# LazyLatte/vortex-raytracing

Hardware: AMD Instinct MI355X
Metric: Mrays/s (primary+shadow) at 1920x1080, 1M-tri BVH (higher is better)
Workload: dtype f32; 1 GPU; configs[2]: Sponza-class 1048576 tris, 1920x1080, primary + 1 shadow ray per hit; frames_in_flight=2, frames_per_launch_group=5, parallelism=1 GPU: whole frames, 5 per set of launches (vxrt_render_batch), 2 sets in flight, world_size=1, bvh_nodes=726809, bvh_depth=13

## Files before the change

vortex-raytracing_amd/csrc/rt_accel.hip:

```cpp
#include <algorithm>
#include <cmath>
#include <cstdio>
#include <cstdlib>
#include <cstring>
#include <utility>
#include "rt_internal.h"
#include "bvh_quant.h"

__global__ void accel_nodes_kernel(const uint32_t* __restrict__ ref, uint32_t n_nodes, uint4* __restrict__ out, int is_tlas,
                                   const uint32_t* __restrict__ bases, const uint32_t* __restrict__ ends, uint32_t nb,
                                   uint32_t n_tris, uint32_t n_blas, uint32_t bias, uint32_t* status) {
  const uint32_t i = blockIdx.x * blockDim.x + threadIdx.x;
  if (i >= n_nodes) return;
  const uint32_t* w = ref + (size_t)i * RT_NODE_DWORDS;
  const uint32_t imask = w[3] >> 24, leftFirst = w[4], leafData = w[5];
  uint32_t base = 0, end = n_nodes;
  if (!is_tlas) {
    bool in = false;
    for (uint32_t j = 0; j < nb; ++j) if (i >= bases[j] && i < ends[j]) { base = bases[j]; end = ends[j]; in = true; }
    if (!in) return;
  }
  if (imask != (is_tlas ? 1u : 0u)) return;
  const bool leaf = is_tlas ? (leafData != 0xffffffffu) : (leafData != 0u);
  if (leaf) return;
// ... 491 lines not shown
      ok = hipGetLastError() == hipSuccess && hipStreamSynchronize(st) == hipSuccess &&
           hipMemcpy(&levels, d_depth + nc, 4, hipMemcpyDeviceToHost) == hipSuccess;
    }
    (void)hipFree(d_depth);
  }
  (void)hipFree(d_ranges); (void)hipFree(d_status); (void)hipFree(d_troot);
  if (!ok || (hstatus & STATUS_BAD_SCENE) != 0) { accel_free(a); return -1; }
  static const int shallow_env = [] { const char* e = getenv("VXRT_SHALLOW"); return e ? atoi(e) : -1; }();
  a->levels = levels;
  a->shallow = levels <= RT_SHALLOW_LEVELS && shallow_env != 0;
  a->dev.nodes_c = (const uint4*)a->nodes_c; a->dev.ref_tlas = (const uint32_t*)s->tlas; a->dev.n_tlas = s->n_tlas_nodes; a->dev.tri_w = (const float4*)a->tri_w;
  a->dev.blas_root = (const uint32_t*)a->blas_root; a->dev.tlas_root = troot;
  a->dev.ident_root = 0u;
  if (troot >= 0xC0000000u && troot < DESC_IDLE) {
    float m[12];
    static const bool ident_off = [] { const char* e = getenv("VXRT_IDENT_ROOT"); return e && e[0] == '0'; }();
    if (!ident_off && hipMemcpy(m, (const uint32_t*)s->blas + (size_t)(troot & PAYLOAD_MASK) * (RT_BLAS_STRIDE / 4) + 1, sizeof m, hipMemcpyDeviceToHost) == hipSuccess) {
      bool id = true;
      for (int i = 0; i < 12; ++i) id = id && m[i] == ((i % 5 == 0) ? 1.0f : 0.0f);
      a->dev.ident_root = id ? 1u : 0u;
    }
  }
  a->dev.exact_decode = (hstatus & STATUS_FMA_DECODE_DIFFERS) ? 1u : 0u;
  a->dev.ref_bvh = (const uint32_t*)s->bvh;
  a->dev.blas = (const uint32_t*)s->blas; a->dev.triEx = (const rt_triex_t*)s->triEx;
  a->dev.mat = (const rt_material_t*)s->mat; a->dev.tex = (const uint8_t*)s->tex;
  a->dev.top_img = (const uint4*)a->top_img; a->dev.n_top = n_top; a->dev.tlas_root_top = troot_top;
  a->dev.blas_root_top = n_top ? a->top_roots + 2 : (const uint32_t*)a->blas_root;
  if (getenv("VXRT_DEBUG")) fprintf(stderr, "[vxrt] accel: %u top-of-tree nodes staged for LDS (cap %u)\n", n_top, TOP_CAP);
  *out = a;
  return 0;
}

int vxrt_accel_destroy(vxrt_accel_t* a) {
  if (!a) return 0;
  accel_free(a);
  return 0;
}

uint64_t vxrt_accel_bytes(const vxrt_accel_t* a) {
  if (!a) return 0;
  return (uint64_t)a->ref.n_tlas_nodes * CNODE_VEC4 * 16 + (uint64_t)a->ref.n_bvh_nodes * CNODE_VEC4 * 16 +
         (uint64_t)a->ref.n_tris * WTRI_FLOATS * 4 + (uint64_t)a->ref.n_blas * 4;
}

int vxrt_accel_info(const vxrt_accel_t* a, uint32_t which, uint64_t* value) {
  if (!a || !value) return -1;
  switch (which) {
  case 0: *value = a->levels; return 0;
  case 1: *value = a->shallow ? 1u : 0u; return 0;
  case 2: *value = a->dev.ident_root; return 0;
  case 3: *value = a->dev.exact_decode; return 0;
  case 4: *value = a->alpha_on ? 1u : 0u; return 0;
  }
  return -1;
}

__global__ __launch_bounds__(256) void accel_alpha_tri_kernel(const rt_triex_t* __restrict__ triEx, uint32_t n_tris, const uint8_t* __restrict__ thr, uint32_t n_mats,
                                                             uint8_t* __restrict__ out) {
  const uint32_t t = blockIdx.x * blockDim.x + threadIdx.x;
  if (t >= n_tris) return;
  const uint32_t m = triEx[t].texId;
  out[t] = m < n_mats ? thr[m] : (uint8_t)0;
}

int vxrt_accel_set_alpha_test(vxrt_accel_t* a, const uint8_t* thresholds, uint32_t n_mats, void* stream) {
  hipStream_t st = (hipStream_t)stream;
  if (!a || a->stale) return -1;
  const vxrt_scene_t& s = a->ref;
  bool any = false;
  if (thresholds) {
    if (n_mats != s.n_mats) return -1;
    for (uint32_t m = 0; m < n_mats; ++m) any = any || thresholds[m] != 0;
  }
  if (any) {
    if (!s.triEx || !s.mat || !s.tex) return -1;
    std::vector<rt_material_t> mats(n_mats);
    if (hipStreamSynchronize(st) != hipSuccess || hipMemcpy(mats.data(), s.mat, (size_t)n_mats * sizeof(rt_material_t), hipMemcpyDeviceToHost) != hipSuccess) return -1;
    for (uint32_t m = 0; m < n_mats; ++m)
      if (thresholds[m] != 0 && mats[m].diffuse_tex_id < 0) return -1;
    if (!a->alpha_mat && hipMalloc((void**)&a->alpha_mat, std::max<size_t>(s.n_mats, 16)) != hipSuccess) return -1;
    if (!a->alpha_tri && hipMalloc((void**)&a->alpha_tri, std::max<size_t>(s.n_tris, 16)) != hipSuccess) return -1;
  }
  for (uint32_t k = 0; k < MAX_FRAMES_IN_FLIGHT; ++k) {
    FrameCtx& c = a->ctx[k];
    if (!c.busy || c.last_stream == st) continue;
    if (c.done_recorded) { if (hipStreamWaitEvent(st, c.ev_done, 0) != hipSuccess) return -1; }
    else if (hipDeviceSynchronize() != hipSuccess) return -1;
  }
  if (any) {
    if (hipMemcpyAsync(a->alpha_mat, thresholds, n_mats, hipMemcpyHostToDevice, st) != hipSuccess) return -1;
    hipLaunchKernelGGL(accel_alpha_tri_kernel, dim3((s.n_tris + 255) / 256), dim3(256), 0, st, (const rt_triex_t*)s.triEx, s.n_tris,
                       (const uint8_t*)a->alpha_mat, n_mats, a->alpha_tri);
    if (hipGetLastError() != hipSuccess) { a->alpha_on = false; (void)hipStreamSynchronize(st); return -1; }
  }
  if (hipStreamSynchronize(st) != hipSuccess) { a->alpha_on = false; return -1; }
  a->alpha_on = any;
  return 0;
}

int vxrt_accel_frames_in_flight(vxrt_accel_t* a, uint32_t n) {
  if (!a || n < 1 || n > MAX_FRAMES_IN_FLIGHT) return -1;
  if (hipDeviceSynchronize() != hipSuccess) return -1;
  a->n_ctx = n; a->next_ctx = 0;
  return 0;
}
// ... 180 lines not shown
```

vortex-raytracing_amd/csrc/rt_internal.h:

```cpp
#pragma once
#include <hip/hip_runtime.h>
#include <stdint.h>
#include <vector>
#include "rt_types.h"
#include "../../include/vortex_hip.h"

#define STATUS_STACK_OVERFLOW 1u
#define STATUS_ITER_LIMIT 2u
#define STATUS_BAD_SCENE 4u
#define STATUS_FMA_DECODE_DIFFERS 8u

struct SceneDev {
  const uint4* nodes_c;
  const uint32_t* ref_tlas;
  uint32_t n_tlas;
  const float4* tri_w;
  const uint32_t* blas_root;
  uint32_t tlas_root;
  uint32_t exact_decode;
  const uint32_t* ref_bvh;
  const uint32_t* blas;
  const rt_triex_t* triEx;
  const rt_material_t* mat;
  const uint8_t* tex;
// ... 14 lines not shown
  uint64_t hitbuf_pixels = 0;
  uint32_t* defer = nullptr;
  uint64_t defer_cap = 0;
  uint32_t* ctl = nullptr;
  ShadeParams* pbatch = nullptr;
  float* cam = nullptr; uint64_t cam_floats = 0;
  bool ctl_dirty = false;
  struct Level {
    float* rays = nullptr; HitRec* hits = nullptr; uint32_t* parent = nullptr; float4* term = nullptr; float* col = nullptr;
    float* srays = nullptr; float* stmax = nullptr; HitRec* shits = nullptr;
    uint64_t cap = 0; uint32_t n = 0;
  };
  std::vector<Level> lv;
  uint32_t* bcount = nullptr;
  struct Lpt { uint32_t* cost = nullptr; uint32_t* order = nullptr; uint32_t cap = 0; uint32_t key[6] = {0, 0, 0, 0, 0, 0}; bool valid = false; };
  Lpt lpt[VXRT_MAX_BATCH + 1];
  float4* ao_geo = nullptr; float4* ao_nrm = nullptr; float4* ao_col = nullptr; uint32_t* ao_cnt = nullptr;
  uint32_t* ao_list = nullptr; uint32_t* ao_hdr = nullptr;
  float* ao_rays = nullptr; float* ao_tmax = nullptr; HitRec* ao_hits = nullptr; uint64_t ao_cap = 0, ao_ray_cap = 0;
  uint32_t* bin_hist = nullptr; uint32_t* bin_keys = nullptr; uint32_t* bin_order = nullptr; uint64_t bin_cap = 0, bin_ray_cap = 0;
  void* pool_spill = nullptr; uint64_t pool_spill_bytes = 0;
  hipStream_t side = nullptr;
  hipEvent_t ev_in = nullptr, ev_side = nullptr, ev_done = nullptr;
  bool busy = false, inited = false, done_recorded = false;
  hipStream_t last_stream = nullptr;
};

struct vxrt_accel {
  SceneDev dev{};
  vxrt_scene_t ref{};
  void* nodes_c = nullptr; void* tri_w = nullptr; void* blas_root = nullptr;
  void* top_img = nullptr; uint32_t* top_roots = nullptr;
  FrameCtx ctx[MAX_FRAMES_IN_FLIGHT];
  uint32_t n_ctx = 1, next_ctx = 0;
  bool stream_seen = false, multi_stream = false; hipStream_t first_stream = nullptr;
  float* uvtab = nullptr;
  uint32_t uv_w = 0, uv_h = 0;
  uint32_t* apriori = nullptr;
  uint32_t* batch_order[VXRT_MAX_BATCH + 1] = {}; uint32_t bo_tiles = 0;
  uint32_t ap_count = 0, ap_key[6] = {0, 0, 0, 0, 0, 0};
  uint64_t ap_cap = 0;
  float max_reflectivity = 0.0f;
  unsigned long long* trace_wave_log = nullptr;
  unsigned long long* end_log = nullptr;
  uint32_t levels = 0;
  bool shallow = false;
  int device = 0;
  struct RefitPlan* refit = nullptr;
  uint32_t blas_status = 0;
  bool stale = false;
  uint8_t* alpha_mat = nullptr; uint8_t* alpha_tri = nullptr;
  bool alpha_on = false;
};
```

vortex-raytracing_amd/csrc/rt_kernels.hip:

```cpp
#include <hip/hip_runtime.h>
#include <stdint.h>
#include "rt_internal.h"
#include "pinhole.h"

__device__ __forceinline__ float std_min(float a, float b) { return (b < a) ? b : a; }
__device__ __forceinline__ float std_max(float a, float b) { return (a < b) ? b : a; }

template <bool EXACT>
__device__ __forceinline__ float slab_interval(float tx1, float tx2, float ty1, float ty2, float tz1, float tz2) {
  float tmin, tmax;
  if (EXACT) {
    tmin = std_min(tx1, tx2);
    tmax = std_max(tx1, tx2);
    tmin = std_max(tmin, std_min(ty1, ty2));
    tmax = std_min(tmax, std_max(ty1, ty2));
    tmin = std_max(tmin, std_min(tz1, tz2));
    tmax = std_min(tmax, std_max(tz1, tz2));
  } else {
    tmin = fmaxf(fmaxf(fminf(tx1, tx2), fminf(ty1, ty2)), fminf(tz1, tz2));
    tmax = fminf(fminf(fmaxf(tx1, tx2), fmaxf(ty1, ty2)), fmaxf(tz1, tz2));
  }
  return (tmax < tmin || tmax <= 0) ? RT_LARGE_FLOAT : tmin;
}

// ... 342 lines not shown
#ifndef RT_QUEUE_DRY_MASK
#define RT_QUEUE_DRY_MASK 1
#endif
#ifndef RT_STEAL_SPREAD
#define RT_STEAL_SPREAD 0
#endif
#ifndef QUEUE_SHARDS
#define QUEUE_SHARDS 8u
#endif
#define QUEUE_STRIDE 32u
#define CTL_QUEUE_DWORDS (QUEUE_SHARDS * QUEUE_STRIDE)
#define CTL_DWORDS (32u + 3u * CTL_QUEUE_DWORDS)
#ifndef RT_WAVES_TRACE
#define RT_WAVES_TRACE 7
#endif
#ifndef RT_LDS_STACK_TRACE
#define RT_LDS_STACK_TRACE 7
#endif
#ifndef RT_WAVES_RENDER
#define RT_WAVES_RENDER 7
#endif
#ifndef RT_LDS_STACK_RENDER
#define RT_LDS_STACK_RENDER 6
#endif
#ifndef RT_WAVES_RENDER_PACKED
#define RT_WAVES_RENDER_PACKED 8
#endif
#ifndef RT_LDS_STACK_RENDER_PACKED
#define RT_LDS_STACK_RENDER_PACKED 5
#endif
#ifndef LDS_STACK
#define LDS_STACK 8
#endif
#ifndef RT_WG_WAVES
#define RT_WG_WAVES 4
#endif
#define RT_WG_THREADS (64 * RT_WG_WAVES)

enum { JOB_RENDER = 0, JOB_RENDER_SHADOW = 1, JOB_TRACE = 2, JOB_RENDER_GI = 3, JOB_TRACE_UNORDERED = 4 };
__host__ __device__ constexpr bool is_trace_job(int job) { return job == JOB_TRACE || job == JOB_TRACE_UNORDERED; }
enum { JOB_CAM = 8 };
__host__ __device__ constexpr int job_base(int job) { return job & ~JOB_CAM; }
__host__ __device__ constexpr bool is_cam_job(int job) { return (job & JOB_CAM) != 0; }
#ifndef RT_WAVES_GI
#define RT_WAVES_GI 7
#endif
#ifndef RT_LDS_STACK_GI
#define RT_LDS_STACK_GI 6
#endif
#ifndef RT_GI_DEAD_MAX
#define RT_GI_DEAD_MAX 64
#endif

#ifdef RT_ISA_MARKS
#define RT_MARK(name) asm volatile("; RTMARK " name)
#else
#define RT_MARK(name)
#endif

__device__ __forceinline__ size_t hit_index(uint32_t x, uint32_t lr, uint32_t tiles_x) {
  return ((size_t)(lr >> 3) * tiles_x + (x >> 3)) * 64u + ((lr & 7u) << 3) + (x & 7u);
}
__device__ __forceinline__ uint32_t frame_row(uint32_t lr, uint32_t y0, uint32_t row_step) { return y0 + (lr >> 3) * row_step + (lr & 7u); }

struct FastDiv { uint32_t d, m, s; };
static FastDiv fast_div_make(uint32_t d) {
  FastDiv f{d ? d : 1u, 1u, 0u};
  while ((1ull << f.s) < f.d) ++f.s;
  f.m = (uint32_t)((((1ull << f.s) - f.d) << 32) / f.d) + 1u;
  return f;
}
__device__ __forceinline__ uint32_t fast_div(uint32_t x, const FastDiv& f) { return (__umulhi(x, f.m) + x) >> f.s; }

struct PersistArgs {
  uint32_t W, H, y0, y1, tiles_x;
  FastDiv div_tiles_x, div_frame_tiles;
  uint32_t row_step;
  uint32_t total;
  const uint32_t* total_dev;
  HitRec* hits;
  const float* rays; const float* tmax; int any_hit;
  const uint32_t* order;
  unsigned long long* counters;
  uint32_t* status;
  uint32_t* queue;
  uint32_t per_shard;
  const float* utab; const float* vtab;
  uint32_t* defer_count; uint32_t* defer_list; uint32_t defer_cap;
  const uint32_t* tile_order; uint32_t* tile_cost;
  uint32_t shard_rot;
  unsigned long long* wave_log;
  unsigned long long* end_log;
  const ShadeParams* pbatch; uint32_t frame_tiles;
  uint32_t* dst; float* colors; uint32_t gi_seed;
  const uint8_t* alpha_tri;
};

#define RT_FAST_INV_MAX 0x1p+64f
#define RT_FAST_POS_MAX 0x1p+60f
__device__ __forceinline__ bool ray_in_fast_domain(float ox, float oy, float oz, float ix, float iy, float iz) {
  return fabsf(ix) <= RT_FAST_INV_MAX && fabsf(iy) <= RT_FAST_INV_MAX && fabsf(iz) <= RT_FAST_INV_MAX && ix != 0.0f && iy != 0.0f && iz != 0.0f &&
         fabsf(ox) <= RT_FAST_POS_MAX && fabsf(oy) <= RT_FAST_POS_MAX && fabsf(oz) <= RT_FAST_POS_MAX;
}

__device__ __forceinline__ float vmax_nonan(float a, float b) { float r; asm("v_max_f32 %0, %1, %2" : "=v"(r) : "v"(a), "v"(b)); return r; }

#define F_FOUND 1u
#define F_ANYHIT 2u
#define F_SHADOW 8u
#define F_WORLD 16u
#define F_RESUMED 32u

template <int JOB, int STATS, bool LDEXP, bool EXACT, bool PACKED = false, bool SHALLOW = false, bool ALPHA = false>
__global__ __launch_bounds__(EXACT ? 256 : RT_WG_THREADS, EXACT ? 4 : (is_trace_job(JOB) ? RT_WAVES_TRACE : (job_base(JOB) == JOB_RENDER_GI ? RT_WAVES_GI : (PACKED ? RT_WAVES_RENDER_PACKED : RT_WAVES_RENDER)))) void rt_persistent_kernel(SceneDev sc, ShadeParams p, PersistArgs A) {
  static_assert(!ALPHA || (STATS == 0 && !PACKED && !SHALLOW && job_base(JOB) != JOB_RENDER_GI), "alpha instantiations: see ALPHA above");
  constexpr int LSTK = EXACT ? LDS_STACK : (is_trace_job(JOB) ? RT_LDS_STACK_TRACE : (job_base(JOB) == JOB_RENDER_GI ? RT_LDS_STACK_GI : (PACKED ? RT_LDS_STACK_RENDER_PACKED : RT_LDS_STACK_RENDER)));
  constexpr int WG_WAVES = EXACT ? 4 : RT_WG_WAVES;
  constexpr bool USE_TOP = RT_TOP_NODES > 0 && !EXACT && !LDEXP;
  constexpr uint32_t DEAD_MAX = is_trace_job(JOB) ? RT_TRACE_DEAD_MAX : (job_base(JOB) == JOB_RENDER_GI ? RT_GI_DEAD_MAX : RT_DEAD_MAX);
  constexpr uint32_t FINISH_MIN = job_base(JOB) == JOB_RENDER_SHADOW ? RT_SHADOW_FINISH_MIN : 65u;
  const uint32_t lane = threadIdx.x & 63u;
  const uint32_t n_jobs = EXACT ? min(*A.defer_count, A.defer_cap) : (A.total_dev ? min(*A.total_dev, A.total) : A.total);
  const uint32_t per_shard = (EXACT || A.total_dev) ? (((n_jobs + QUEUE_SHARDS - 1) / QUEUE_SHARDS + 63u) & ~63u) : A.per_shard;

  __shared__ uint2 s_stk[WG_WAVES][LSTK][64];
  constexpr int NCTX = (!EXACT && is_trace_job(JOB)) ? 8 : 9;
  __shared__ uint32_t s_ctx[WG_WAVES][NCTX][64];
  __shared__ uint32_t s_dry;
  if (threadIdx.x == 0) s_dry = 0u;
  float* s_cam = nullptr;
  if constexpr (is_cam_job(JOB)) {
    s_cam = cam_lds<CAM_TAB>();
    for (uint32_t i = threadIdx.x; i < (uint32_t)CAM_TAB; i += blockDim.x) s_cam[i] = A.utab[i];
  }
  __syncthreads();
  uint2* const lstk = &s_stk[threadIdx.x >> 6][0][lane];
  uint32_t* const ctx = &s_ctx[threadIdx.x >> 6][0][lane];
#define CTX(i) ctx[((NCTX == 8 && (i) > 5) ? (i) - 1 : (i)) * 64]
  __shared__ uint4 s_top[USE_TOP ? 4 : 1][USE_TOP ? RT_TOP_NODES : 1];
  constexpr bool TRI_LDS = RT_TRI_LDS > 0 && !EXACT && !is_trace_job(JOB);
  __shared__ float4 s_tri[TRI_LDS ? WG_WAVES : 1][TRI_LDS ? 3 * RT_TRI_LDS : 1];
  const uint32_t n_top = USE_TOP ? min(sc.n_top, (uint32_t)RT_TOP_NODES) : 0u;
  if (USE_TOP && n_top) {
    for (uint32_t i = threadIdx.x; i < 4u * n_top; i += (uint32_t)(64 * WG_WAVES)) s_top[i / n_top][i % n_top] = sc.top_img[(size_t)(i / n_top) * RT_TOP_NODES + (i % n_top)];
    __syncthreads();
  }
  const uint32_t root_desc = (USE_TOP && n_top) ? sc.tlas_root_top : sc.tlas_root;
  const uint32_t* const blas_roots = (USE_TOP && n_top) ? sc.blas_root_top : sc.blas_root;
  const uint32_t root_blas_desc = is_inst_desc(root_desc) ? blas_roots[root_desc & PAYLOAD_MASK] : DESC_DONE;

  float arx = 0, ary = 0, arz = 0, aix = 0, aiy = 0, aiz = 0;
  float hitd = 0, path_m = 0, tos_m = 0;
  uint32_t cur = DESC_IDLE, tos_d = DESC_DONE, job = 0, flags = 0;
  float g_col[3] = {0.f, 0.f, 0.f}, g_alb[3] = {0.f, 0.f, 0.f}, g_ray[6] = {0.f, 0.f, 0.f, 0.f, 0.f, 0.f};
  int sp = 0;
  constexpr int STACK_CAP = SHALLOW ? 3 * RT_SHALLOW_LEVELS : LSTK + RT_STACK_ENTRIES;
  static_assert(STACK_CAP > LSTK, "stack");
  uint32_t ovf_d[STACK_CAP - LSTK];
  float ovf_m[STACK_CAP - LSTK];
  bool queue_empty = false;
  const uint32_t xcc_id = RT_XCC_HOME ? (uint32_t)__builtin_amdgcn_s_getreg((3 << 11) | (0 << 6) | 20) : blockIdx.x;
  const uint32_t shard = (xcc_id + A.shard_rot) % QUEUE_SHARDS;
  uint32_t tries = 0, loc_next = 0, loc_end = 0;
  uint32_t loc_off = 0;
  uint32_t lpt_tile = 0xFFFFFFFFu, lpt_work = 0; unsigned long long lpt_t0 = 0;
  Fetches fx;
  unsigned nrays = 0, nhit = 0;
  unsigned long long t_first = 0;
// ... 70 lines not shown
    for (int i = 0; i < 13; ++i) bw[i] = bp[i];
    if (STATS) { fx.node++; fx.inst++; }
    const float m00 = __uint_as_float(bw[1]), m01 = __uint_as_float(bw[2]), m02 = __uint_as_float(bw[3]), m03 = __uint_as_float(bw[4]);
    const float m10 = __uint_as_float(bw[5]), m11 = __uint_as_float(bw[6]), m12 = __uint_as_float(bw[7]), m13 = __uint_as_float(bw[8]);
    const float m20 = __uint_as_float(bw[9]), m21 = __uint_as_float(bw[10]), m22 = __uint_as_float(bw[11]), m23 = __uint_as_float(bw[12]);
    arx = m00 * ox + m01 * oy + m02 * oz + m03;
    ary = m10 * ox + m11 * oy + m12 * oz + m13;
    arz = m20 * ox + m21 * oy + m22 * oz + m23;
    const float cdx = m00 * dx + m01 * dy + m02 * dz;
    const float cdy = m10 * dx + m11 * dy + m12 * dz;
    const float cdz = m20 * dx + m21 * dy + m22 * dz;
    aix = 1.0f / cdx; aiy = 1.0f / cdy; aiz = 1.0f / cdz;
    const bool s2 = ray_in_fast_domain(arx, ary, arz, aix, aiy, aiz);
    if (!EXACT && !s2) { defer(true); return; }
    flags &= ~F_WORLD;
    CTX(0) = __float_as_uint(cdx); CTX(1) = __float_as_uint(cdy); CTX(2) = __float_as_uint(cdz);
    CTX(8) = blasIdx;
    cur = blas_roots[blasIdx];
  };
  auto start_ray = [&](float ox, float oy, float oz, float dx, float dy, float dz, float tmax_, bool any_) {
    arx = ox; ary = oy; arz = oz;
    aix = 1.0f / dx; aiy = 1.0f / dy; aiz = 1.0f / dz;
    const bool safe = ray_in_fast_domain(ox, oy, oz, aix, aiy, aiz);
    flags = (flags & (F_SHADOW | F_RESUMED)) | F_WORLD | (any_ ? F_ANYHIT : 0u);
    if (!EXACT && !safe) {
      if (!is_trace_job(JOB) && !is_cam_job(JOB) && !(flags & F_SHADOW)) cur = DESC_IDLE; else defer(false);
      return;
    }
    hitd = tmax_ > RT_LARGE_FLOAT ? RT_LARGE_FLOAT : tmax_;
    path_m = -__builtin_inff(); sp = 0; tos_d = DESC_DONE;
    cur = root_desc;
    nrays++;
    if (is_inst_desc(root_desc)) {
      const bool no_neg_zero = __float_as_uint(ox) != 0x80000000u && __float_as_uint(oy) != 0x80000000u && __float_as_uint(oz) != 0x80000000u;
      if (sc.ident_root && safe && no_neg_zero) {
        if (STATS) { fx.node++; fx.inst++; }
        flags &= ~F_WORLD;
        CTX(0) = __float_as_uint(dx); CTX(1) = __float_as_uint(dy); CTX(2) = __float_as_uint(dz);
        CTX(8) = root_desc & PAYLOAD_MASK;
        cur = root_blas_desc;
      } else enter_instance(root_desc & PAYLOAD_MASK, ox, oy, oz, dx, dy, dz);
    }
  };
  volatile uint32_t* const vovf_d = ovf_d;
  volatile float* const vovf_m = ovf_m;
  auto push = [&](uint32_t d, float m) {
    if (tos_d != DESC_DONE) {
      if (sp < LSTK) lstk[sp * 64] = make_uint2(tos_d, __float_as_uint(tos_m));
      else { ovf_d[sp - LSTK] = tos_d; ovf_m[sp - LSTK] = tos_m; }
      ++sp;
    }
    tos_d = d; tos_m = m;
  };
  auto pop_next = [&]() {
    cur = DESC_DONE;
    while (tos_d != DESC_DONE) {
      const uint32_t d = tos_d;
      const float m = tos_m;
      if (sp > 0) {
        --sp;
        if (sp < LSTK) { const uint2 e = lstk[sp * 64]; tos_d = e.x; tos_m = __uint_as_float(e.y); }
        else { tos_d = ovf_d[sp - LSTK]; tos_m = ovf_m[sp - LSTK]; }
      } else {
        tos_d = DESC_DONE;
      }
      if (m < hitd) { cur = d; path_m = m; break; }
    }
  };

  for (;;) {
    RT_MARK("fetch");
    if (STATS && A.wave_log) wl_tmark = __builtin_readcyclecounter();
    {
      const unsigned long long idle = __ballot(cur == DESC_IDLE);
      if (!queue_empty && idle != 0ull && (is_trace_job(JOB) || FINISH_MIN > 64u || idle == ~0ull || RT_DEAD_MAX < 64)) {
        const uint32_t wl_tries0 = tries; const unsigned long long wl_tpoll0 = (STATS && A.wave_log) ? __builtin_readcyclecounter() : 0ull;
        if (loc_next == loc_end) {
          uint32_t dry = RT_QUEUE_DRY_MASK ? *(volatile uint32_t*)&s_dry : 0u;
          while (tries < QUEUE_SHARDS) {
            const uint32_t step = RT_STEAL_SPREAD ? (((tries & 1u) << 2) | (tries & 2u) | ((tries >> 2) & 1u)) : tries;
            const uint32_t sid = (shard + step) % QUEUE_SHARDS;
            if (RT_QUEUE_DRY_MASK && ((dry >> sid) & 1u)) { ++tries; continue; }
            const uint32_t s_lo = sid * per_shard;
            uint32_t in_range;
            asm volatile("s_cmp_lt_u32 %1, %2\n\ts_cselect_b32 %0, 1, 0 ; RTGUARD shard_range" : "=s"(in_range)
                         : "s"(__builtin_amdgcn_readfirstlane(s_lo)), "s"(__builtin_amdgcn_readfirstlane(n_jobs)) : "scc");
            if (!in_range) { ++tries; continue; }
            const uint32_t s_n = min(per_shard, n_jobs - s_lo);
            uint32_t base = 0;
            constexpr uint32_t CHUNK = (is_trace_job(JOB) && !EXACT) ? (uint32_t)RT_TRACE_CHUNK : (uint32_t)RT_CHUNK;
            if (lane == 0) base = atomicAdd(A.queue + sid * QUEUE_STRIDE, CHUNK);
            base = __shfl(base, 0);
            if (base < s_n) {
              loc_next = s_lo + base; loc_end = s_lo + min(base + CHUNK, s_n);
              break;
            }
            if (RT_QUEUE_DRY_MASK) {
              if (lane == 0) atomicOr(&s_dry, 1u << sid);
              dry |= 1u << sid;
            }
            ++tries;
          }
          if (tries >= QUEUE_SHARDS) { queue_empty = true; if (STATS && A.wave_log && !wl_tq) wl_tq = wall_clock64(); }
          if (STATS && A.wave_log && !USE_TOP && tries != wl_tries0 && lane == 0) wl_no23 += (unsigned)(__builtin_readcyclecounter() - wl_tpoll0);
        }
        uint32_t avail = loc_end - loc_next;
        if (!is_trace_job(JOB) && !EXACT) {
// ... 23 lines not shown
            job = loc_next + rank + loc_off;
            flags = 0;
            if (!EXACT && is_trace_job(JOB) && A.order) job = A.order[job];
            if (EXACT) {
              const uint32_t wd = A.defer_list[job];
              job = wd & 0x7fffffffu;
              if (wd >> 31) { flags = F_SHADOW | F_RESUMED; if (job_base(JOB) == JOB_RENDER_SHADOW) CTX(5) = __float_as_uint(hit_slot()->dist); }
            }
            float ox, oy, oz, dx, dy, dz, tm;
            if (is_trace_job(JOB)) {
              world_ray(ox, oy, oz, dx, dy, dz, tm);
              start_ray(ox, oy, oz, dx, dy, dz, tm, A.any_hit != 0);
            } else {
              uint32_t x, y;
              pixel_of(job, x, y);
              if (x < A.W && y < A.y1) {
                world_ray(ox, oy, oz, dx, dy, dz, tm);
                start_ray(ox, oy, oz, dx, dy, dz, tm, (flags & F_SHADOW) != 0u);
              }
            }
          }
        }
        loc_next += min(avail, (uint32_t)__popcll(idle));
      }
      if (__ballot(cur != DESC_IDLE) == 0ull) {
        if (queue_empty && loc_next == loc_end) {
          if (!is_trace_job(JOB) && !EXACT && A.tile_cost && lane == 0 && lpt_tile != 0xFFFFFFFFu) {
            A.tile_cost[lpt_tile] = lpt_work;
            if (STATS && A.wave_log) A.tile_cost[2u * (A.total >> 6) + lpt_tile] = (uint32_t)min(wall_clock64() - lpt_t0, 0xFFFFFFFFull);
          }
          break;
        }
        if (STATS && A.wave_log) wl_tf += __builtin_readcyclecounter() - wl_tmark;
        continue;
      }
    }
    if (STATS && A.wave_log) wl_tf += __builtin_readcyclecounter() - wl_tmark;

    for (;;) {
      RT_MARK("loop_top");
      if (!is_trace_job(JOB) && !EXACT) ++lpt_work;
      if (STATS && A.wave_log) {
        const unsigned long long nm = __ballot(is_node_desc(cur));
        ++wl_iter;
        if (nm) {
          ++wl_node_x; wl_node_l += (unsigned)__popcll(nm);
          const uint32_t c0 = __shfl(cur, __ffsll((long long)nm) - 1);
          if (__ballot(is_node_desc(cur) && cur == c0) == nm) ++wl_no3;
        }
      }
      if (STATS && A.wave_log) wl_t0 = __builtin_readcyclecounter();
      RT_MARK("node");
      if (is_node_desc(cur)) {
        const bool top = (cur >> 30) == DK_TLAS;
        if (top && !(flags & F_WORLD)) {
          float ox, oy, oz, dx, dy, dz, tm;
          world_ray(ox, oy, oz, dx, dy, dz, tm);
          arx = ox; ary = oy; arz = oz; aix = 1.0f / dx; aiy = 1.0f / dy; aiz = 1.0f / dz;
          flags |= F_WORLD;
        }
        const uint32_t ni = cur & PAYLOAD_MASK;
        uint4 q0, q1, q2, q3;
        if (USE_TOP && (cur & DESC_TOP_FLAG)) {
          typedef uint32_t u32x4_t __attribute__((ext_vector_type(4)));
          typedef __attribute__((address_space(3))) const volatile u32x4_t lds_u32x4_t;
          lds_u32x4_t* tp = (lds_u32x4_t*)&s_top[0][0] + (cur & DESC_TOP_SLOT);
          const u32x4_t t0 = tp[0], t1 = tp[RT_TOP_NODES], t2 = tp[2 * RT_TOP_NODES], t3 = tp[3 * RT_TOP_NODES];
          q0 = make_uint4(t0.x, t0.y, t0.z, t0.w); q1 = make_uint4(t1.x, t1.y, t1.z, t1.w);
          q2 = make_uint4(t2.x, t2.y, t2.z, t2.w); q3 = make_uint4(t3.x, t3.y, t3.z, t3.w);
          if (STATS && A.wave_log) ++wl_no23;
        } else {
          const uint4* np = sc.nodes_c + (size_t)ni * CNODE_VEC4;
          q0 = np[0]; q1 = np[1]; q2 = np[2]; q3 = np[3];
        }
        const uint32_t* ref_node = nullptr;
        if (LDEXP) ref_node = top ? sc.ref_tlas + (size_t)ni * RT_NODE_DWORDS : sc.ref_bvh + (size_t)(ni - sc.n_tlas) * RT_NODE_DWORDS;
        if (STATS) fx.node++;
        Cand c[4];
        eval_children<EXACT, LDEXP>(q0, q1, q2, q3, ref_node, arx, ary, arz, aix, aiy, aiz, hitd, c);
        if (((job_base(JOB) == JOB_RENDER_SHADOW && RT_UNORDERED_OCCLUSION) || JOB == JOB_TRACE_UNORDERED) && STATS != 1 && __all((flags & F_ANYHIT) != 0u)) {
          const bool v0 = c[0].d < __builtin_inff(), v1 = c[1].d < __builtin_inff(), v2 = c[2].d < __builtin_inff(), v3 = c[3].d < __builtin_inff();
          if (v0 || v1 || v2 || v3) {
            bool more = true;
            if (sp + 4 > STACK_CAP) { atomicOr(A.status, STATUS_STACK_OVERFLOW); more = false; }
            cur = v0 ? c[0].desc : (v1 ? c[1].desc : (v2 ? c[2].desc : c[3].desc));
            if (more) {
              if (v1 && v0) push(c[1].desc, c[1].d);
              if (v2 && (v0 || v1)) push(c[2].desc, c[2].d);
              if (v3 && (v0 || v1 || v2)) push(c[3].desc, c[3].d);
            }
          } else {
            pop_next();
          }
        } else {
          order_children(c);
          if (c[0].d < __builtin_inff()) {
            bool more = true;
            if (sp + 4 > STACK_CAP) { atomicOr(A.status, STATUS_STACK_OVERFLOW); more = false; }
            if (more && c[3].d < __builtin_inff()) push(c[3].desc, vmax_nonan(path_m, c[3].d));
            if (more && c[2].d < __builtin_inff()) push(c[2].desc, vmax_nonan(path_m, c[2].d));
            if (more && c[1].d < __builtin_inff()) push(c[1].desc, vmax_nonan(path_m, c[1].d));
            cur = c[0].desc;
            path_m = vmax_nonan(path_m, c[0].d);
          } else {
            pop_next();
          }
        }
      }
      if (STATS && A.wave_log) { const unsigned long long t1 = __builtin_readcyclecounter(); wl_tn += t1 - wl_t0; wl_t0 = t1; }
      RT_MARK("inst");
      if (__any(is_inst_desc(cur))) {
        if (is_inst_desc(cur)) {
          float ox, oy, oz, dx, dy, dz, tm;
          world_ray(ox, oy, oz, dx, dy, dz, tm);
          enter_instance(cur & PAYLOAD_MASK, ox, oy, oz, dx, dy, dz);
        }
      }
      RT_MARK("leaf");
      const unsigned long long leafm = __ballot(is_leaf_desc(cur));
      if (leafm != 0ull && ((uint32_t)__popcll(leafm) >= (is_trace_job(JOB) ? RT_TRACE_LEAF_MIN : RT_LEAF_MIN) || __ballot(is_node_desc(cur) || is_inst_desc(cur)) == 0ull)) {
        if (STATS && A.wave_log) { ++wl_leaf_x; wl_leaf_l += (unsigned)__popcll(leafm); }
        if (!is_trace_job(JOB) && !EXACT) lpt_work += 2u;
        {
          bool tri_from_lds = false;
          if (TRI_LDS) {
            const uint32_t L0 = __shfl(cur, __ffsll((long long)leafm) - 1);
            const uint32_t c0 = (L0 >> LEAF_FIRST_BITS) & LEAF_MAX_INLINE;
            const unsigned long long same = __ballot(cur == L0);
            if (c0 != 0u && c0 <= (uint32_t)RT_TRI_LDS && (uint32_t)__popcll(same) >= (uint32_t)RT_TRI_LDS_MIN) {
              if (lane < 3u * c0) s_tri[threadIdx.x >> 6][lane] = sc.tri_w[(size_t)(L0 & LEAF_FIRST_MASK) * 3 + lane];
              tri_from_lds = cur == L0;
              if (STATS && A.wave_log) wl_no23 += (unsigned)__popcll(same);
            }
          }
          if (is_leaf_desc(cur)) {
            if (STATS) fx.node++;
            uint32_t leftFirst = cur & LEAF_FIRST_MASK, triCount = (cur >> LEAF_FIRST_BITS) & LEAF_MAX_INLINE;
            if (triCount == 0u) {
              const uint32_t* rn = sc.ref_bvh + (size_t)leftFirst * RT_NODE_DWORDS;
              leftFirst = rn[4]; triCount = rn[5];
            }
            const float cdx = __uint_as_float(CTX(0)), cdy = __uint_as_float(CTX(1)), cdz = __uint_as_float(CTX(2));
            bool stop = false;
            constexpr bool PREFETCH = is_trace_job(JOB) && RT_TRI_PREFETCH;
            float4 n0 = make_float4(0.f, 0.f, 0.f, 0.f), n1 = n0, n2 = n0;
            if (PREFETCH) { const float4* tp0 = sc.tri_w + (size_t)leftFirst * 3; n0 = tp0[0]; n1 = tp0[1]; n2 = tp0[2]; }
            for (uint32_t i = 0; i < triCount; ++i) {
              const uint32_t triIdx = leftFirst + i;
              float4 t0, t1, t2;
              if (TRI_LDS && tri_from_lds) {
                typedef float f32x4_t __attribute__((ext_vector_type(4)));
                typedef __attribute__((address_space(3))) const volatile f32x4_t lds_f32x4_t;
                lds_f32x4_t* lp = (lds_f32x4_t*)&s_tri[threadIdx.x >> 6][0] + 3u * i;
                const f32x4_t a0 = lp[0], a1 = lp[1], a2 = lp[2];
                t0 = make_float4(a0.x, a0.y, a0.z, a0.w); t1 = make_float4(a1.x, a1.y, a1.z, a1.w); t2 = make_float4(a2.x, a2.y, a2.z, a2.w);
              } else
              if (PREFETCH) {
                t0 = n0; t1 = n1; t2 = n2;
                if (i + 1u < triCount) { const float4* tn = sc.tri_w + (size_t)(triIdx + 1u) * 3; n0 = tn[0]; n1 = tn[1]; n2 = tn[2]; }
              } else {
                const float4* tp = sc.tri_w + (size_t)triIdx * 3;
                t0 = tp[0]; t1 = tp[1]; t2 = tp[2];
              }
              if (STATS) fx.tri++;
              float bx, by, bz;
              const float d = ray_tri(arx, ary, arz, cdx, cdy, cdz, t0, t1, t2, bx, by, bz);
              if (d < hitd) {
                if constexpr (ALPHA) { if (alpha_rejects(sc, A.alpha_tri, triIdx, bx, by, bz)) continue; }
                hitd = d;
                flags |= F_FOUND;
                if (!(job_base(JOB) == JOB_RENDER_SHADOW && (flags & F_SHADOW))) { CTX(3) = __float_as_uint(bx); CTX(4) = __float_as_uint(by); CTX(6) = CTX(8); CTX(7) = triIdx; }
                if (flags & F_ANYHIT) { stop = true; break; }
                if (!(path_m < hitd)) break;
              }
            }
            if (stop) { sp = 0; tos_d = DESC_DONE; cur = DESC_DONE; }
            else pop_next();
          }
        }
      }
      if (STATS && A.wave_log) { const unsigned long long t1 = __builtin_readcyclecounter(); wl_tl += t1 - wl_t0; }
      RT_MARK("loop_exit");
      const unsigned long long work = __ballot(is_work_desc(cur));
      if (work == 0ull) break;
      const unsigned long long done = __ballot(cur == DESC_DONE);
      const uint32_t n_done = (uint32_t)__popcll(done);
      const uint32_t n_idle = queue_empty && loc_next == loc_end ? 0u : 64u - (uint32_t)__popcll(work | done);
      if (n_done + n_idle >= DEAD_MAX || n_done >= FINISH_MIN) break;
    }

    RT_MARK("finish");
    if (STATS && A.wave_log) wl_tmark = __builtin_readcyclecounter();
    if (cur == DESC_DONE) {
      const bool found = (flags & F_FOUND) != 0u;
      HitRec h; h.dist = RT_LARGE_FLOAT; h.bx = 0; h.by = 0; h.bz = 0; h.blasIdx = 0; h.triIdx = 0;
      if (is_trace_job(JOB)) {
        if (found) {
          h.dist = hitd; h.bx = __uint_as_float(CTX(3)); h.by = __uint_as_float(CTX(4)); h.bz = 1 - h.bx - h.by;
          h.blasIdx = CTX(6); h.triIdx = CTX(7);
        }
        if (RT_TRACE_NT) {
          uint32_t* hp = (uint32_t*)hit_slot();
          __builtin_nontemporal_store(__float_as_uint(h.dist), hp); __builtin_nontemporal_store(__float_as_uint(h.bx), hp + 1);
          __builtin_nontemporal_store(__float_as_uint(h.by), hp + 2); __builtin_nontemporal_store(__float_as_uint(h.bz), hp + 3);
          __builtin_nontemporal_store(h.blasIdx, hp + 4); __builtin_nontemporal_store(h.triIdx, hp + 5);
        } else *hit_slot() = h;
        cur = DESC_IDLE;
      } else if (job_base(JOB) == JOB_RENDER_GI) {
        uint32_t x, y;
        pixel_of(job, x, y);
        const size_t e = (size_t)x + (size_t)y * A.W;
        bool write = false;
        float cr = 0.f, cg = 0.f, cb = 0.f;
        if (found) {
          h.dist = hitd; h.bx = __uint_as_float(CTX(3)); h.by = __uint_as_float(CTX(4)); h.bz = 1 - h.bx - h.by;
          h.blasIdx = CTX(6); h.triIdx = CTX(7);
        }
        if (!(flags & F_SHADOW)) {
          float ox, oy, oz, dx, dy, dz;
          pixel_ray(x, y, ox, oy, oz, dx, dy, dz);
          if (!found) {
            cr = p.bg[0]; cg = p.bg[1]; cb = p.bg[2];
            write = true;
          } else {
            float r, g, b, refl, Ix, Iy, Iz, Nx, Ny, Nz, a3[3];
            shade_terms<false>(sc, p, ox, oy, oz, dx, dy, dz, h, false, r, g, b, refl, Ix, Iy, Iz, Nx, Ny, Nz, nullptr, a3);
            float thr = 1.0f;
            thr *= refl;
            g_col[0] = r + p.bg[0] * thr; g_col[1] = g + p.bg[1] * thr; g_col[2] = b + p.bg[2] * thr;
            g_alb[0] = a3[0]; g_alb[1] = a3[1]; g_alb[2] = a3[2];
            ao_sample_ray(x, y, A.W, 1u, 0u, A.gi_seed, Ix, Iy, Iz, Nx, Ny, Nz, dx, dy, dz, g_ray);
            flags = F_SHADOW;
            start_ray(g_ray[0], g_ray[1], g_ray[2], g_ray[3], g_ray[4], g_ray[5], RT_LARGE_FLOAT, false);
          }
        } else {
          float r, g, b;
          shade_eval<false>(sc, p, g_ray[0], g_ray[1], g_ray[2], g_ray[3], g_ray[4], g_ray[5], h, found, false, r, g, b);
// ... 1244 lines not shown
    if (!upload_batch(a, c, r, t, s)) return false;
    A.pbatch = c->pbatch; A.tile_order = a->batch_order[r.batch];
  }
  if (!grow_device({{(void**)&c->defer, sizeof(uint32_t)}}, &c->defer_cap, A.total, GrowSync::STREAM, s)) return false;
  A.defer_count = c->ctl; A.defer_list = c->defer; A.defer_cap = A.total;
  A.queue = c->ctl + 32;
  A.per_shard = ((A.total + QUEUE_SHARDS - 1) / QUEUE_SHARDS + 63u) & ~63u;
  A.shard_rot = host_knobs().shard_rot;
  A.alpha_tri = a->alpha_on ? a->alpha_tri : nullptr;
  if (lpt && !ensure_lpt_tables(c, r, n_tiles, A, s)) return false;
  return r.cams || ensure_apriori(a, r, t, s);
}

struct LaunchPlan {
  bool lpt;
  bool packed;
  bool side_launch;
  uint32_t side_wgs;
  bool side_reserve;
  uint32_t grid_div;
  bool grid_div_small;
};
static LaunchPlan launch_plan(const vxrt_accel* a, const RenderRequest& r, uint32_t n_tiles, bool lpt, uint32_t ap_count) {
  const HostKnobs& k = host_knobs();
  LaunchPlan plan;
  plan.lpt = lpt;
  plan.packed = k.packed >= 0 ? k.packed != 0 : ((a->n_ctx > 1 || (k.packed_batch && r.batch > 1)) && n_tiles >= LPT_MIN_TILES);
  plan.side_launch = ap_count != 0;
  plan.side_wgs = plan.side_launch ? std::min<uint32_t>(EXACT_GRID, (ap_count + 255u) / 256u) : 0u;
  plan.side_reserve = k.side_reserve >= 0 ? k.side_reserve != 0 : a->n_ctx == 1;
  plan.grid_div = k.grid_div > 0 ? (uint32_t)k.grid_div : ((k.grid_div == 0 && a->n_ctx > 1) ? a->n_ctx : 1u);
  plan.grid_div_small = k.grid_div == 0;
  return plan;
}

template <class K>
static uint32_t main_grid(K kernel, const LaunchPlan& plan, uint32_t total) {
  const uint32_t side_wgs_r = plan.side_reserve ? plan.side_wgs : 0u;
  uint32_t g = persistent_grid(kernel, total + (uint64_t)side_wgs_r * RT_WG_THREADS);
  const uint32_t cap = persistent_grid(kernel, ~0ull >> 8);
  const uint32_t div = (plan.grid_div_small && (uint64_t)total >= 2ull * 64ull * RT_WG_WAVES * cap) ? 1u : plan.grid_div;
  if (div > 1u) g = std::min<uint32_t>(g, std::max<uint32_t>(cap / div, 1u));
  return std::max<uint32_t>(1u, g > side_wgs_r ? g - side_wgs_r : 1u);
}

struct FrameLaunch {
  const vxrt_accel* a; FrameCtx* c; const LaunchPlan& plan; const ShadeParams& p; hipStream_t s;
  PersistArgs A, X, X0;
};

template <int JOB, int STATS, bool PACKED, bool ALPHA = false>
static void launch_traversal(const FrameLaunch& l) {
  static_assert(!(PACKED && (job_base(JOB) == JOB_RENDER_GI || STATS != 0)), "only the timed render jobs have a packed form");
  with_decode_and_depth<STATS == 0 && !ALPHA>(l.a, [&](auto ld, auto sh) {
    const auto k_main = rt_persistent_kernel<JOB, STATS, decltype(ld)::value, false, PACKED, decltype(sh)::value, ALPHA>;
    const auto k_exact = rt_persistent_kernel<JOB, STATS, decltype(ld)::value, true, false, false, ALPHA>;
    if (l.plan.side_launch) hipLaunchKernelGGL(k_exact, dim3(l.plan.side_wgs), dim3(256), 0, l.c->side, l.a->dev, l.p, l.X0);
    hipLaunchKernelGGL(k_main, dim3(main_grid(k_main, l.plan, l.A.total)), dim3(RT_WG_THREADS), 0, l.s, l.a->dev, l.p, l.A);
    hipLaunchKernelGGL(k_exact, dim3(EXACT_GRID), dim3(256), 0, l.s, l.a->dev, l.p, l.X);
  });
}
template <int STATS, bool PACKED, int CAM = 0, bool ALPHA = false>
static void launch_render(bool shadow, const FrameLaunch& l) {
  if (shadow) launch_traversal<JOB_RENDER_SHADOW | CAM, STATS, PACKED, ALPHA>(l); else launch_traversal<JOB_RENDER | CAM, STATS, PACKED, ALPHA>(l);
}

static bool traverse_frame(vxrt_accel* a, FrameCtx* c, const RenderRequest& r, const LaunchPlan& plan, const ShadeParams& p, const PersistArgs& A, hipStream_t s) {
  FrameLaunch l{a, c, plan, p, s, A, A, A};
  l.X.queue = c->ctl + 32 + CTL_QUEUE_DWORDS;
  c->ctl_dirty = true;
  if (plan.side_launch) {
    const bool drained = hipStreamQuery(s) == hipSuccess;
    if (!drained && (hipEventRecord(c->ev_in, s) != hipSuccess || hipStreamWaitEvent(c->side, c->ev_in, 0) != hipSuccess)) return false;
    const uint32_t ap_count = a->ap_count * r.batch;
    l.X0.queue = c->ctl + 32 + 2 * CTL_QUEUE_DWORDS;
    l.X0.defer_count = a->apriori; l.X0.defer_list = a->apriori + 1; l.X0.defer_cap = ap_count;
  }
  if (gi_fused_frame(r)) {
    for (PersistArgs* g : {&l.A, &l.X, &l.X0}) { g->dst = r.dst; g->colors = r.colors; g->gi_seed = r.ao->seed; }
    if (r.cams) launch_traversal<JOB_RENDER_GI | JOB_CAM, 0, false>(l); else launch_traversal<JOB_RENDER_GI, 0, false>(l);
  }
  else if (l.A.alpha_tri) { if (r.cams) launch_render<0, false, JOB_CAM, true>(r.shadow != 0, l); else launch_render<0, false, 0, true>(r.shadow != 0, l); }
  else if (r.counting == Counting::TIMED_TRAVERSAL) launch_render<2, false>(r.shadow != 0, l);
  else if (r.counting == Counting::REFERENCE_ORDER) launch_render<1, false>(r.shadow != 0, l);
  else if (r.cams)      launch_render<0, false, JOB_CAM>(r.shadow != 0, l);
  else if (plan.packed) launch_render<0, true>(r.shadow != 0, l);
  else                  launch_render<0, false>(r.shadow != 0, l);
  return !plan.side_launch || (hipEventRecord(c->ev_side, c->side) == hipSuccess && hipStreamWaitEvent(s, c->ev_side, 0) == hipSuccess);
}

static bool shade_frame(vxrt_accel* a, FrameCtx* c, const RenderRequest& r, const Tiles& t, bool lpt_sort, const ShadeParams& p, const PersistArgs& A, hipStream_t s) {
  const FrameCtx::Lpt& L = c->lpt[r.batch];
  const uint32_t n_tiles = (uint32_t)t.total, n_rows = t.y * 8u;
  const uint64_t npx = (uint64_t)r.width * n_rows * r.batch;
  const uint32_t lpt_blocks = lpt_sort ? QUEUE_SHARDS : 0u;
  const dim3 sgrid((uint32_t)((npx + 255) / 256) + lpt_blocks), block(256);
  const uint32_t* base_order = r.batch > 1 ? (const uint32_t*)a->batch_order[r.batch] : (const uint32_t*)nullptr;
  if (r.cams) {
    hipLaunchKernelGGL(r.batch > 1 ? rt_shade_camera_kernel<true> : rt_shade_camera_kernel<false>, sgrid, block, 0, s, a->dev, p, r.width, r.height, r.y0, r.y1, t.row_step,
                       n_rows, (const float*)A.utab, (const HitRec*)c->hitbuf, r.dst, (HitRec*)r.hits, r.colors, c->ctl, lpt_blocks, (const uint32_t*)L.cost,
                       L.order, n_tiles, A.per_shard >> 6, r.batch, (const ShadeParams*)c->pbatch, r.dst_frame_stride, base_order);
  } else {
    const bool stats = r.counting != Counting::TIMED;
    hipLaunchKernelGGL(stats ? rt_shade_kernel<true> : rt_shade_kernel<false>, sgrid, block, 0, s, a->dev, p, r.width, r.height, r.y0, r.y1, t.row_step,
                       n_rows, A.utab, A.vtab, (const HitRec*)c->hitbuf, r.dst, (HitRec*)r.hits, r.colors, r.counters, c->ctl, lpt_blocks, (const uint32_t*)L.cost,
                       L.order, n_tiles, A.per_shard >> 6, stats ? 1u : r.batch, stats ? (const ShadeParams*)nullptr : (const ShadeParams*)c->pbatch,
                       stats ? (uint64_t)0 : r.dst_frame_stride, base_order);
  }
  return hipGetLastError() == hipSuccess;
}

static int render_common(vxrt_accel_t* a, const RenderRequest& r) {
// ... 330 lines not shown
```

Before: 11170 Mrays/s.

## Add identity-root kernel specialization, batched stack pushes, and cheaper loop-exit check

Adds an IDENT template variant of the persistent traversal kernel. When the scene has an identity root (shallow, no exact decode, no alpha), this variant drops the TLAS and instance handling at compile time. It also replaces the sequential per-child stack pushes with one batched push that writes all pending entries at once, and a pop that skips culled entries while keeping the top of stack in registers. The loop-exit ballot work is skipped when few lanes are idle. Together these are meant to cut branching and LDS traffic per node, at the cost of more kernel instantiations and more complex stack logic that could be subtly wrong at overflow boundaries.

```diff
diff --git a/vortex-raytracing_amd/csrc/rt_accel.hip b/vortex-raytracing_amd/csrc/rt_accel.hip
--- a/vortex-raytracing_amd/csrc/rt_accel.hip
+++ b/vortex-raytracing_amd/csrc/rt_accel.hip
@@ -567,6 +567,7 @@
   case 2: *value = a->dev.ident_root; return 0;
   case 3: *value = a->dev.exact_decode; return 0;
   case 4: *value = a->alpha_on ? 1u : 0u; return 0;
+  case 5: *value = ident_root_form(a) ? 1u : 0u; return 0;
   }
   return -1;
 }
diff --git a/vortex-raytracing_amd/csrc/rt_internal.h b/vortex-raytracing_amd/csrc/rt_internal.h
--- a/vortex-raytracing_amd/csrc/rt_internal.h
+++ b/vortex-raytracing_amd/csrc/rt_internal.h
@@ -90,3 +90,10 @@
   uint8_t* alpha_mat = nullptr; uint8_t* alpha_tri = nullptr;
   bool alpha_on = false;
 };
+
+#ifndef RT_IDENT_ROOT_KERNEL
+#define RT_IDENT_ROOT_KERNEL 1
+#endif
+static inline bool ident_root_form(const vxrt_accel* a) {
+  return RT_IDENT_ROOT_KERNEL && a->dev.ident_root != 0u && a->shallow && !a->dev.exact_decode && !a->alpha_on;
+}
diff --git a/vortex-raytracing_amd/csrc/rt_kernels.hip b/vortex-raytracing_amd/csrc/rt_kernels.hip
--- a/vortex-raytracing_amd/csrc/rt_kernels.hip
+++ b/vortex-raytracing_amd/csrc/rt_kernels.hip
@@ -418,6 +418,10 @@
 #define RT_GI_DEAD_MAX 64
 #endif
 
+#ifndef RT_BATCH_PUSH
+#define RT_BATCH_PUSH 1
+#endif
+
 #ifdef RT_ISA_MARKS
 #define RT_MARK(name) asm volatile("; RTMARK " name)
 #else
@@ -477,9 +481,10 @@
 #define F_WORLD 16u
 #define F_RESUMED 32u
 
-template <int JOB, int STATS, bool LDEXP, bool EXACT, bool PACKED = false, bool SHALLOW = false, bool ALPHA = false>
+template <int JOB, int STATS, bool LDEXP, bool EXACT, bool PACKED = false, bool SHALLOW = false, bool ALPHA = false, bool IDENT = false>
 __global__ __launch_bounds__(EXACT ? 256 : RT_WG_THREADS, EXACT ? 4 : (is_trace_job(JOB) ? RT_WAVES_TRACE : (job_base(JOB) == JOB_RENDER_GI ? RT_WAVES_GI : (PACKED ? RT_WAVES_RENDER_PACKED : RT_WAVES_RENDER)))) void rt_persistent_kernel(SceneDev sc, ShadeParams p, PersistArgs A) {
   static_assert(!ALPHA || (STATS == 0 && !PACKED && !SHALLOW && job_base(JOB) != JOB_RENDER_GI), "alpha instantiations: see ALPHA above");
+  static_assert(!IDENT || (STATS == 0 && !ALPHA && !EXACT && !LDEXP && SHALLOW && (job_base(JOB) == JOB_RENDER || job_base(JOB) == JOB_RENDER_SHADOW)), "identity-root instantiations: see IDENT above");
   constexpr int LSTK = EXACT ? LDS_STACK : (is_trace_job(JOB) ? RT_LDS_STACK_TRACE : (job_base(JOB) == JOB_RENDER_GI ? RT_LDS_STACK_GI : (PACKED ? RT_LDS_STACK_RENDER_PACKED : RT_LDS_STACK_RENDER)));
   constexpr int WG_WAVES = EXACT ? 4 : RT_WG_WAVES;
   constexpr bool USE_TOP = RT_TOP_NODES > 0 && !EXACT && !LDEXP;
@@ -656,7 +661,58 @@
     }
     tos_d = d; tos_m = m;
   };
+  auto push_pending = [&](bool p0, uint32_t d0, float m0, bool p1, uint32_t d1, float m1, bool p2, uint32_t d2, float m2) {
+    if (!RT_BATCH_PUSH) {
+      if (p0) push(d0, m0);
+      if (p1) push(d1, m1);
+      if (p2) push(d2, m2);
+      return;
+    }
+    if (!(p0 || p1 || p2)) return;
+    const bool w_top = tos_d != DESC_DONE;
+    const bool w0 = p0 && (p1 || p2), w1 = p1 && p2;
+    const int q0 = sp + (w_top ? 1 : 0), q1 = q0 + (w0 ? 1 : 0), end = q1 + (w1 ? 1 : 0);
+    if (end <= LSTK) {
+      if (w_top) lstk[sp * 64] = make_uint2(tos_d, __float_as_uint(tos_m));
+      if (w0) lstk[q0 * 64] = make_uint2(d0, __float_as_uint(m0));
+      if (w1) lstk[q1 * 64] = make_uint2(d1, __float_as_uint(m1));
+    } else if (sp >= LSTK) {
+      if (w_top) { ovf_d[sp - LSTK] = tos_d; ovf_m[sp - LSTK] = tos_m; }
+      if (w0) { ovf_d[q0 - LSTK] = d0; ovf_m[q0 - LSTK] = m0; }
+      if (w1) { ovf_d[q1 - LSTK] = d1; ovf_m[q1 - LSTK] = m1; }
+    } else {
+      auto put = [&](int q, uint32_t d, float m) {
+        if (q < LSTK) lstk[q * 64] = make_uint2(d, __float_as_uint(m));
+        else { ovf_d[q - LSTK] = d; ovf_m[q - LSTK] = m; }
+      };
+      if (w_top) put(sp, tos_d, tos_m);
+      if (w0) put(q0, d0, m0);
+      if (w1) put(q1, d1, m1);
+    }
+    sp = end;
+    tos_d = p2 ? d2 : (p1 ? d1 : d0);
+    tos_m = p2 ? m2 : (p1 ? m1 : m0);
+  };
+  auto stack_load = [&](int i, uint32_t& d, float& m) {
+    typedef uint32_t u32x2_t __attribute__((ext_vector_type(2)));
+    typedef __attribute__((address_space(3))) const u32x2_t lds_u32x2_t;
+    if (i < LSTK) { const u32x2_t e = ((lds_u32x2_t*)lstk)[i * 64]; d = e.x; m = __uint_as_float(e.y); }
+    else { d = ovf_d[i - LSTK]; m = ovf_m[i - LSTK]; }
+  };
   auto pop_next = [&]() {
+    if (RT_BATCH_PUSH) {
+      uint32_t d = tos_d; float m = tos_m;
+      while (d != DESC_DONE && !(m < hitd)) {
+        if (sp > 0) { --sp; stack_load(sp, d, m); } else d = DESC_DONE;
+      }
+      cur = d;
+      tos_d = DESC_DONE;
+      if (d != DESC_DONE) {
+        path_m = m;
+        if (sp > 0) { --sp; stack_load(sp, tos_d, tos_m); }
+      }
+      return;
+    }
     cur = DESC_DONE;
     while (tos_d != DESC_DONE) {
       const uint32_t d = tos_d;
@@ -786,7 +842,7 @@
       if (STATS && A.wave_log) wl_t0 = __builtin_readcyclecounter();
       RT_MARK("node");
       if (is_node_desc(cur)) {
-        const bool top = (cur >> 30) == DK_TLAS;
+        const bool top = !IDENT && (cur >> 30) == DK_TLAS;
         if (top && !(flags & F_WORLD)) {
           float ox, oy, oz, dx, dy, dz, tm;
           world_ray(ox, oy, oz, dx, dy, dz, tm);
@@ -812,17 +868,14 @@
         if (STATS) fx.node++;
         Cand c[4];
         eval_children<EXACT, LDEXP>(q0, q1, q2, q3, ref_node, arx, ary, arz, aix, aiy, aiz, hitd, c);
+        RT_MARK("stack");
         if (((job_base(JOB) == JOB_RENDER_SHADOW && RT_UNORDERED_OCCLUSION) || JOB == JOB_TRACE_UNORDERED) && STATS != 1 && __all((flags & F_ANYHIT) != 0u)) {
           const bool v0 = c[0].d < __builtin_inff(), v1 = c[1].d < __builtin_inff(), v2 = c[2].d < __builtin_inff(), v3 = c[3].d < __builtin_inff();
           if (v0 || v1 || v2 || v3) {
             bool more = true;
             if (sp + 4 > STACK_CAP) { atomicOr(A.status, STATUS_STACK_OVERFLOW); more = false; }
             cur = v0 ? c[0].desc : (v1 ? c[1].desc : (v2 ? c[2].desc : c[3].desc));
-            if (more) {
-              if (v1 && v0) push(c[1].desc, c[1].d);
-              if (v2 && (v0 || v1)) push(c[2].desc, c[2].d);
-              if (v3 && (v0 || v1 || v2)) push(c[3].desc, c[3].d);
-            }
+            push_pending(more && v1 && v0, c[1].desc, c[1].d, more && v2 && (v0 || v1), c[2].desc, c[2].d, more && v3 && (v0 || v1 || v2), c[3].desc, c[3].d);
           } else {
             pop_next();
           }
@@ -831,9 +884,8 @@
           if (c[0].d < __builtin_inff()) {
             bool more = true;
             if (sp + 4 > STACK_CAP) { atomicOr(A.status, STATUS_STACK_OVERFLOW); more = false; }
-            if (more && c[3].d < __builtin_inff()) push(c[3].desc, vmax_nonan(path_m, c[3].d));
-            if (more && c[2].d < __builtin_inff()) push(c[2].desc, vmax_nonan(path_m, c[2].d));
-            if (more && c[1].d < __builtin_inff()) push(c[1].desc, vmax_nonan(path_m, c[1].d));
+            push_pending(more && c[3].d < __builtin_inff(), c[3].desc, vmax_nonan(path_m, c[3].d), more && c[2].d < __builtin_inff(), c[2].desc, vmax_nonan(path_m, c[2].d),
+                         more && c[1].d < __builtin_inff(), c[1].desc, vmax_nonan(path_m, c[1].d));
             cur = c[0].desc;
             path_m = vmax_nonan(path_m, c[0].d);
           } else {
@@ -843,7 +895,7 @@
       }
       if (STATS && A.wave_log) { const unsigned long long t1 = __builtin_readcyclecounter(); wl_tn += t1 - wl_t0; wl_t0 = t1; }
       RT_MARK("inst");
-      if (__any(is_inst_desc(cur))) {
+      if (!IDENT && __any(is_inst_desc(cur))) {
         if (is_inst_desc(cur)) {
           float ox, oy, oz, dx, dy, dz, tm;
           world_ray(ox, oy, oz, dx, dy, dz, tm);
@@ -852,7 +904,7 @@
       }
       RT_MARK("leaf");
       const unsigned long long leafm = __ballot(is_leaf_desc(cur));
-      if (leafm != 0ull && ((uint32_t)__popcll(leafm) >= (is_trace_job(JOB) ? RT_TRACE_LEAF_MIN : RT_LEAF_MIN) || __ballot(is_node_desc(cur) || is_inst_desc(cur)) == 0ull)) {
+      if (leafm != 0ull && ((uint32_t)__popcll(leafm) >= (is_trace_job(JOB) ? RT_TRACE_LEAF_MIN : RT_LEAF_MIN) || __ballot(is_node_desc(cur) || (!IDENT && is_inst_desc(cur))) == 0ull)) {
         if (STATS && A.wave_log) { ++wl_leaf_x; wl_leaf_l += (unsigned)__popcll(leafm); }
         if (!is_trace_job(JOB) && !EXACT) lpt_work += 2u;
         {
@@ -917,6 +969,7 @@
       RT_MARK("loop_exit");
       const unsigned long long work = __ballot(is_work_desc(cur));
       if (work == 0ull) break;
+      if (RT_BATCH_PUSH && 64u - (uint32_t)__popcll(work) < (DEAD_MAX < FINISH_MIN ? DEAD_MAX : FINISH_MIN)) continue;
       const unsigned long long done = __ballot(cur == DESC_DONE);
       const uint32_t n_done = (uint32_t)__popcll(done);
       const uint32_t n_idle = queue_empty && loc_next == loc_end ? 0u : 64u - (uint32_t)__popcll(work | done);
@@ -2267,12 +2320,20 @@
 template <int JOB, int STATS, bool PACKED, bool ALPHA = false>
 static void launch_traversal(const FrameLaunch& l) {
   static_assert(!(PACKED && (job_base(JOB) == JOB_RENDER_GI || STATS != 0)), "only the timed render jobs have a packed form");
-  with_decode_and_depth<STATS == 0 && !ALPHA>(l.a, [&](auto ld, auto sh) {
-    const auto k_main = rt_persistent_kernel<JOB, STATS, decltype(ld)::value, false, PACKED, decltype(sh)::value, ALPHA>;
-    const auto k_exact = rt_persistent_kernel<JOB, STATS, decltype(ld)::value, true, false, false, ALPHA>;
+  const auto launch = [&](auto k_main, auto k_exact) {
     if (l.plan.side_launch) hipLaunchKernelGGL(k_exact, dim3(l.plan.side_wgs), dim3(256), 0, l.c->side, l.a->dev, l.p, l.X0);
     hipLaunchKernelGGL(k_main, dim3(main_grid(k_main, l.plan, l.A.total)), dim3(RT_WG_THREADS), 0, l.s, l.a->dev, l.p, l.A);
     hipLaunchKernelGGL(k_exact, dim3(EXACT_GRID), dim3(256), 0, l.s, l.a->dev, l.p, l.X);
+  };
+  if constexpr (RT_IDENT_ROOT_KERNEL && STATS == 0 && !ALPHA && job_base(JOB) != JOB_RENDER_GI) {
+    if (ident_root_form(l.a)) {
+      launch(rt_persistent_kernel<JOB, 0, false, false, PACKED, true, false, true>, rt_persistent_kernel<JOB, 0, false, true, false, false, false>);
+      return;
+    }
+  }
+  with_decode_and_depth<STATS == 0 && !ALPHA>(l.a, [&](auto ld, auto sh) {
+    launch(rt_persistent_kernel<JOB, STATS, decltype(ld)::value, false, PACKED, decltype(sh)::value, ALPHA>,
+           rt_persistent_kernel<JOB, STATS, decltype(ld)::value, true, false, false, ALPHA>);
   });
 }
 template <int STATS, bool PACKED, int CAM = 0, bool ALPHA = false>
```

Result: faster. 11710 Mrays/s, median of 6 (+4.8%).
